# CederGroupHub/chgnet

Measured on NVIDIA H100. Metric: structures_per_sec_EFS, higher is better.
Workload: dtype f32

## Files before the change

chgnet_b200/csrc/gated_ws.cu:

```cuda
#include "gated_common.cuh"
#include "tc.cuh"

namespace chg {
namespace gated {
namespace {

constexpr int WS_THREADS = 512;
constexpr int TR = 128;
constexpr int HALF_BYTES = TR * 64 * 4;
constexpr int IMG_BYTES = 64 * 64 * 4;
constexpr int STRIP = 16;

struct WsSmem {
  static constexpr int IMG_OFF = 0;
  static constexpr int HS_OFF = 4 * IMG_BYTES;
  static constexpr int O_OFF = HS_OFF + 2 * HALF_BYTES;
  static constexpr int GIDX_OFF = O_OFF + HALF_BYTES;
  static constexpr int EIDX_OFF = GIDX_OFF + 2 * 3 * TR * 4;
  static constexpr int B2_OFF = EIDX_OFF + 4 * TR * 4;
  static constexpr int LN_OFF = B2_OFF + 128 * 4;
  static constexpr int TOTAL = LN_OFF + 256 * 4;
};

struct WsBars {
  uint64_t a_full[2], a_empty[2];
};

struct FusedArgs {
  const float* p_a;
  const float* p_b;
  const float* p_c;
  const float* wgt;
  const int32_t* idx0;
  const int32_t* idx1;
  const int32_t* idx2;
  const int32_t* ptr;
  int32_t n_rows, n_seg;
  const float* w2t;
  const float* b2;
  const float* ln;
  float* out;
  float* parts;
  float* save_pre;
  float* save_p;
};

__device__ __forceinline__ void prefetch_l2(const void* p) { asm volatile("prefetch.global.L2 [%0];" ::"l"(p)); }
__device__ __forceinline__ int swz(int r, int c) { return r * 256 + ((c ^ (r & 7)) << 4); }

__device__ __forceinline__ void build_image_ws(uint8_t* hi, uint8_t* lo, const float* __restrict__ src, int ld, int col0,
                                               int tid) {
  for (int i = tid; i < 4096; i += (int)blockDim.x) {
    const int kk = i >> 6, n = i & 63;
    uint32_t h, l;
    tc::split_tf32(__ldg(src + (size_t)kk * ld + col0 + n), h, l);
    const uint32_t off = tc::kmajor_offset(n, kk, 64);
    *reinterpret_cast<uint32_t*>(hi + off) = h;
    *reinterpret_cast<uint32_t*>(lo + off) = l;
  }
}

__device__ __forceinline__ float quad_sum(float v) {
  v += __shfl_xor_sync(0xffffffffu, v, 1);
  v += __shfl_xor_sync(0xffffffffu, v, 2);
  return v;
}
__device__ __forceinline__ void bias_ln_frag(float (&d)[32], const float* s_b2, const float* s_gamma, const float* s_beta,
                                             bool use_ln, float* save_rows, int row0, int n_rows) {
#pragma unroll
  for (int i = 0; i < 32; ++i) d[i] += s_b2[tc::frag_col(i)];
  if (save_rows != nullptr) {
#pragma unroll
    for (int i = 0; i < 32; i += 2) {
      const int g = row0 + tc::frag_row(i);
      if (g < n_rows) *reinterpret_cast<float2*>(save_rows + (size_t)g * 128 + tc::frag_col(i)) = make_float2(d[i], d[i + 1]);
    }
  }
  if (!use_ln) return;
#pragma unroll
  for (int h = 0; h < 2; ++h) {
    float s1 = 0.f;
#pragma unroll
    for (int i = 0; i < 32; ++i)
      if (((i >> 1) & 1) == h) s1 += d[i];
    const float mean = quad_sum(s1) * (1.f / 64.f);
    float s2 = 0.f;
#pragma unroll
    for (int i = 0; i < 32; ++i)
      if (((i >> 1) & 1) == h) s2 = fmaf(d[i] - mean, d[i] - mean, s2);
    const float rstd = 1.f / sqrtf(quad_sum(s2) * (1.f / 64.f) + LN_EPS);
#pragma unroll
    for (int i = 0; i < 32; ++i)
      if (((i >> 1) & 1) == h) d[i] = fmaf((d[i] - mean) * rstd, s_gamma[tc::frag_col(i)], s_beta[tc::frag_col(i)]);
  }
}

template <int MODE>
__global__ void __launch_bounds__(WS_THREADS, 1) gated_ws_fwd_kernel(const FusedArgs a) {
  extern __shared__ __align__(1024) uint8_t smem_raw[];
  uint8_t* s_img = smem_raw + WsSmem::IMG_OFF;
  uint8_t* s_hs = smem_raw + WsSmem::HS_OFF;
  uint8_t* s_o = smem_raw + WsSmem::O_OFF;
  int* s_gidx = reinterpret_cast<int*>(smem_raw + WsSmem::GIDX_OFF);
  int* s_eidx = reinterpret_cast<int*>(smem_raw + WsSmem::EIDX_OFF);
  float* s_b2 = reinterpret_cast<float*>(smem_raw + WsSmem::B2_OFF);
  float* s_ln = reinterpret_cast<float*>(smem_raw + WsSmem::LN_OFF);
  __shared__ __align__(8) WsBars bars;

  const int tid = threadIdx.x, warp = tid >> 5, lane = tid & 31;
  const bool use_ln = a.ln != nullptr;
  const int n_tiles = (a.n_rows + TR - 1) / TR;

  build_image_ws(s_img, s_img + IMG_BYTES, a.w2t, 128, 0, tid);
  build_image_ws(s_img + 2 * IMG_BYTES, s_img + 3 * IMG_BYTES, a.w2t, 128, 64, tid);
  if (tid < 128) s_b2[tid] = a.b2[tid];
  if (tid < 256) s_ln[tid] = use_ln ? a.ln[tid] : 0.f;
  if (tid == 0) {
    for (int i = 0; i < 2; ++i) {
      tc::mbar_init(&bars.a_full[i], 128);
      tc::mbar_init(&bars.a_empty[i], 256);
    }
    tc::mbar_fence_init();
  }
  tc::fence_async_smem();
  __syncthreads();

  if (warp >= 8) {
    const int half = (warp - 8) >> 2;
    const int gt = tid - 256 - half * 128;
    const int tx = gt & 15, ty = gt >> 4;
    int* gi = s_gidx + half * 3 * TR;
    uint8_t* stage = s_hs + half * HALF_BYTES;
    const int col = half * 64 + tx * 4;
    constexpr int PB = 4;
    int tl = 0;
    for (int tile = blockIdx.x; tile < n_tiles; tile += gridDim.x, ++tl) {
      const int base = tile * TR;
      {
        const int r = min(base + gt, a.n_rows - 1);
        gi[gt] = a.idx0[r];
        gi[TR + gt] = a.idx1[r];
        gi[2 * TR + gt] = a.idx2[r];
      }
      tc::wg_barrier(1 + half, 128);
      {
        const int nt = tile + gridDim.x;
        if (nt < n_tiles) {
          const int r = min(nt * TR + gt, a.n_rows - 1);
          const float* row = MODE == BOND ? a.p_c + (size_t)r * 128 + half * 64 : a.p_b + (size_t)__ldg(a.idx2 + r) * 128 + half * 64;
          prefetch_l2(row);
          prefetch_l2(row + 32);
        }
      }
#pragma unroll 1
      for (int b = 0; b < 16 / PB; ++b) {
        float4 v[PB];
#pragma unroll
        for (int i = 0; i < PB; ++i) {
          const int row = ty + 8 * (b * PB + i);
          const float* s0 = a.p_a + (size_t)gi[row] * 256 + col;
          const float* s1 = a.p_a + (size_t)gi[TR + row] * 256 + 128 + col;
          const float* s2 = a.p_b + (size_t)gi[2 * TR + row] * 128 + col;
          v[i] = ldg4(s0) + ldg4(s1) + ldg4(s2);
          if (MODE == BOND) v[i] = v[i] + ldg4(a.p_c + (size_t)min(base + row, a.n_rows - 1) * 128 + col);
        }
        if (b == 0) tc::mbar_wait(&bars.a_empty[half], (tl & 1) ^ 1);
#pragma unroll
        for (int i = 0; i < PB; ++i) {
          const int row = ty + 8 * (b * PB + i);
          if (a.save_pre != nullptr && base + row < a.n_rows) stg4(a.save_pre + (size_t)(base + row) * 128 + col, v[i]);
          *reinterpret_cast<float4*>(stage + swz(row, tx)) =
              make_float4(silu_f(v[i].x), silu_f(v[i].y), silu_f(v[i].z), silu_f(v[i].w));
        }
      }
      tc::wg_barrier(1 + half, 128);
      tc::mbar_arrive(&bars.a_full[half]);
    }
  } else {
    const int cw = warp >> 2;
    const int t = tid & 127;
    const int row0 = cw * 64;
    int* s_seg = s_eidx;
    int* s_wrow = s_eidx + TR;
    int* s_sa = s_eidx + 2 * TR;
    int* s_sb = s_eidx + 3 * TR;
    const uint32_t img = tc::smem_u32(s_img);
    int tl = 0;
    for (int tile = blockIdx.x; tile < n_tiles; tile += gridDim.x, ++tl) {
      const int base = tile * TR;
      {
        const int r = min(base + t, a.n_rows - 1);
        if (cw == 0) {
          const int seg = a.idx0[r];
          s_seg[t] = seg;
          s_sa[t] = __ldg(a.ptr + seg);
          s_sb[t] = __ldg(a.ptr + seg + 1);
        } else {
          const int wr = MODE == BOND ? a.idx1[r] : a.idx2[r];
          s_wrow[t] = wr;
          prefetch_l2(a.wgt + (size_t)wr * 64);
          prefetch_l2(a.wgt + (size_t)wr * 64 + 32);
        }
      }
      float dc[32], dg[32];
#pragma unroll
      for (int i = 0; i < 32; ++i) dc[i] = dg[i] = 0.f;
      tc::mbar_wait(&bars.a_full[0], tl & 1);
      tc::wg_gemm_k64<64>(dc, [&](int r, int k) { return *reinterpret_cast<const float*>(s_hs + swz(row0 + r, k >> 2) + (k & 3) * 4); },
                          img, img + IMG_BYTES, 2048);
      tc::mbar_arrive(&bars.a_empty[0]);
      tc::mbar_wait(&bars.a_full[1], tl & 1);
      tc::wg_gemm_k64<64>(dg, [&](int r, int k) { return *reinterpret_cast<const float*>(s_hs + HALF_BYTES + swz(row0 + r, k >> 2) + (k & 3) * 4); },
                          img + 2 * IMG_BYTES, img + 3 * IMG_BYTES, 2048);
      tc::mbar_arrive(&bars.a_empty[1]);
      float* save = a.save_p != nullptr ? a.save_p + (size_t)base * 128 : nullptr;
      bias_ln_frag(dc, s_b2, s_ln, s_ln + 64, use_ln, save, row0, a.n_rows - base);
      bias_ln_frag(dg, s_b2 + 64, s_ln + 128, s_ln + 192, use_ln, save != nullptr ? save + 64 : nullptr, row0, a.n_rows - base);
#pragma unroll
      for (int i = 0; i < 32; i += 2) {
        const int r = row0 + tc::frag_row(i), c = tc::frag_col(i);
        *reinterpret_cast<float2*>(s_o + swz(r, c >> 2) + (c & 3) * 4) =
            make_float2(silu_f(dc[i]) * sigmoid_f(dg[i]), silu_f(dc[i + 1]) * sigmoid_f(dg[i + 1]));
      }
      tc::wg_barrier(3, 256);

      const int strip_lo = base + warp * STRIP;
      const int strip_hi = min(strip_lo + STRIP, a.n_rows);
      if (strip_lo < a.n_rows) {
        float2 w[STRIP];
#pragma unroll
        for (int i = 0; i < STRIP; ++i) {
          const int rr = warp * STRIP + i;
          const float2 w0 = __ldg(reinterpret_cast<const float2*>(a.wgt + (size_t)s_wrow[rr] * 64) + lane);
          if (MODE == ATOM) {
            w[i] = w0;
          } else {
            const float2 wi = __ldg(reinterpret_cast<const float2*>(a.wgt + (size_t)s_seg[rr] * 64) + lane);
            w[i] = make_float2(wi.x * w0.x, wi.y * w0.y);
          }
        }
        float2 acc = make_float2(0.f, 0.f);
        int cur_row = warp * STRIP;
        auto emit = [&](int row0_, const float2& v) {
          const int seg = s_seg[row0_], sa = s_sa[row0_], sb = s_sb[row0_];
          float* dst;
          if (sa >= strip_lo && sb <= strip_hi) {
            dst = a.out + (size_t)seg * 64;
          } else {
            dst = a.parts + ((size_t)(strip_lo / STRIP) * 2 + (sa < strip_lo ? 0 : 1)) * 64;
          }
          *reinterpret_cast<float2*>(dst + lane * 2) = v;
        };
#pragma unroll
        for (int i = 0; i < STRIP; ++i) {
          const int rr = warp * STRIP + i;
          if (strip_lo + i < strip_hi) {
            if (s_seg[rr] != s_seg[cur_row]) {
              emit(cur_row, acc);
              cur_row = rr;
              acc = make_float2(0.f, 0.f);
            }
            const float2 o = *reinterpret_cast<const float2*>(s_o + swz(rr, lane >> 1) + (lane & 1) * 8);
            acc.x = fmaf(o.x, w[i].x, acc.x);
            acc.y = fmaf(o.y, w[i].y, acc.y);
          }
        }
        emit(cur_row, acc);
      }
      tc::wg_barrier(3, 256);
    }
  }
}

__global__ void seg_stitch_kernel(const int32_t* __restrict__ ptr, int n_seg, const float* __restrict__ parts,
                                  float* __restrict__ out) {
  const int idx = blockIdx.x * blockDim.x + threadIdx.x;
  const int s = idx >> 4, l = idx & 15;
  if (s >= n_seg) return;
  const int a = ptr[s], b = ptr[s + 1];
  if (a >= b) {
    stg4(out + (size_t)s * 64 + l * 4, make_float4(0.f, 0.f, 0.f, 0.f));
    return;
  }
  const int k0 = a / STRIP, k1 = (b - 1) / STRIP;
  if (k0 == k1) return;
  float4 acc = ldg4(parts + ((size_t)k0 * 2 + 1) * 64 + l * 4);
  for (int k = k0 + 1; k <= k1; ++k) acc = acc + ldg4(parts + ((size_t)k * 2) * 64 + l * 4);
  stg4(out + (size_t)s * 64 + l * 4, acc);
}

template <int MODE>
int launch_fused(const FusedArgs& a, cudaStream_t stream) {
  if (a.n_seg == 0) return CHG_OK;
  if (a.n_rows > 0) {
    static bool attr_set[MAX_DEVICES] = {};
    bool& set = attr_set[device_ordinal()];
    if (!set) {
      CHG_CUDA(cudaFuncSetAttribute(gated_ws_fwd_kernel<MODE>, cudaFuncAttributeMaxDynamicSharedMemorySize, WsSmem::TOTAL));
      set = true;
    }
    const int n_tiles = (a.n_rows + TR - 1) / TR;
    gated_ws_fwd_kernel<MODE><<<min(n_tiles, sm_count()), WS_THREADS, WsSmem::TOTAL, stream>>>(a);
    cudaError_t e = cudaGetLastError();
    if (e != cudaSuccess) {
      set_error("gated_ws_fwd_kernel: launch failed: %s", cudaGetErrorString(e));
      return CHG_ERR_CUDA;
    }
    count_launch();
  }
  seg_stitch_kernel<<<(a.n_seg * 16 + 255) / 256, 256, 0, stream>>>(a.ptr, a.n_seg, a.parts, a.out);
  CHG_LAUNCH_END();
}

}

int atom_conv_fused_ws(const float* pcn, const float* pe, const float* wag, const int32_t* center, const int32_t* nbr,
                       const int32_t* d2u, const int32_t* ptr_c, int n_edges, int n_atoms, const float* w2t, const float* b2,
                       const float* ln, float* agg, float* save_p, float* parts, cudaStream_t stream) {
  FusedArgs a{pcn, pe, nullptr, wag, center, nbr, d2u, ptr_c, n_edges, n_atoms, w2t, b2, ln, agg, parts, nullptr, save_p};
  return launch_fused<ATOM>(a, stream);
}

int bond_conv_fused_ws(const float* pij, const float* px, const float* pa, const float* wbg, const int32_t* ang_atom,
                       const int32_t* ang_i, const int32_t* ang_j, const int32_t* ptr_i, int n_angles, int n_slots,
                       const float* w2t, const float* b2, const float* ln, float* agg, float* save_pre, float* save_p,
                       float* parts, cudaStream_t stream) {
  FusedArgs a{pij, px, pa, wbg, ang_i, ang_j, ang_atom, ptr_i, n_angles, n_slots, w2t, b2, ln, agg, parts, save_pre, save_p};
  return launch_fused<BOND>(a, stream);
}

}
}

using namespace chg;

extern "C" int64_t chg_gated_fused_workspace_floats(int32_t n_rows) {
  if (n_rows < 0) return -1;
  const int64_t msg = (int64_t)n_rows * 64, parts = ((int64_t)n_rows + 15) / 16 * 128;
  return (msg > parts ? msg : parts) + 64;
}

extern "C" int chg_atom_conv_fused(const float* pcn, const float* pe, const float* wag, const int32_t* center,
                                   const int32_t* nbr, const int32_t* d2u, const int32_t* ptr_c, int32_t n_edges,
                                   int32_t n_atoms, const float* w2t, const float* b2, const float* ln, float* agg,
                                   float* save_p, float* work, void* stream) {
  CHG_CHECK_ARG(n_edges >= 0 && n_atoms >= 0, "negative size");
  if (n_atoms == 0) return CHG_OK;
  CHG_CHECK_ARG(ptr_c && agg, "null pointer");
  CHG_CHECK_ARG(n_edges == 0 || (pcn && pe && wag && center && nbr && d2u && w2t && b2 && work), "null pointer");
  if (gated_impl() == 3 && n_edges >= ws_min_rows())
    return gated::atom_conv_fused_ws(pcn, pe, wag, center, nbr, d2u, ptr_c, n_edges, n_atoms, w2t, b2, ln, agg, save_p, work,
                                     as_stream(stream));
  const int rc = chg_atom_conv_fwd(pcn, pe, wag, center, nbr, d2u, n_edges, w2t, b2, ln, work, save_p, nullptr, stream);
  if (rc != CHG_OK) return rc;
  return chg_segment_sum(work, 64, nullptr, ptr_c, n_atoms, n_edges, 0, agg, 64, stream);
}

extern "C" int chg_bond_conv_fused(const float* pij, const float* px, const float* pa, const float* wbg,
                                   const int32_t* ang_atom, const int32_t* ang_i, const int32_t* ang_j,
                                   const int32_t* ptr_i, int32_t n_angles, int32_t n_slots, const float* w2t,
                                   const float* b2, const float* ln, float* agg, float* save_pre, float* save_p,
                                   float* work, void* stream) {
  CHG_CHECK_ARG(n_angles >= 0 && n_slots >= 0, "negative size");
  if (n_slots == 0) return CHG_OK;
  CHG_CHECK_ARG(ptr_i && agg, "null pointer");
  CHG_CHECK_ARG(n_angles == 0 || (pij && px && pa && wbg && ang_atom && ang_i && ang_j && w2t && b2 && work), "null pointer");
  if (gated_impl() == 3 && n_angles >= ws_min_rows())
    return gated::bond_conv_fused_ws(pij, px, pa, wbg, ang_atom, ang_i, ang_j, ptr_i, n_angles, n_slots, w2t, b2, ln, agg,
                                     save_pre, save_p, work, as_stream(stream));
  const int rc = chg_bond_conv_fwd(pij, px, pa, wbg, ang_atom, ang_i, ang_j, n_angles, w2t, b2, ln, work, save_pre, save_p, stream);
  if (rc != CHG_OK) return rc;
  return chg_segment_sum(work, 64, nullptr, ptr_i, n_slots, n_angles, 0, agg, 64, stream);
}

namespace chg {
namespace gated {
namespace {

struct WsBwdSmem {
  static constexpr int IMG_OFF = 0;
  static constexpr int T1_OFF = 4 * IMG_BYTES;
  static constexpr int T2_OFF = T1_OFF + 2 * HALF_BYTES;
  static constexpr int PIDX_OFF = T2_OFF + 2 * HALF_BYTES;
  static constexpr int FIDX_OFF = PIDX_OFF + 3 * TR * 4;
  static constexpr int LN_OFF = FIDX_OFF + 3 * TR * 4;
  static constexpr int TOTAL = LN_OFF + 256 * 4;
};

struct WsBwdBars {
  uint64_t a_full, a_empty;
};

template <int MODE>
__global__ void __launch_bounds__(WS_THREADS, 1) gated_ws_bwd_kernel(const BwdArgs a) {
  extern __shared__ __align__(1024) uint8_t smem_raw[];
  uint8_t* s_img = smem_raw + WsBwdSmem::IMG_OFF;
  uint8_t* s_t1 = smem_raw + WsBwdSmem::T1_OFF;
  uint8_t* s_t2 = smem_raw + WsBwdSmem::T2_OFF;
  int* s_pidx = reinterpret_cast<int*>(smem_raw + WsBwdSmem::PIDX_OFF);
  int* s_fidx = reinterpret_cast<int*>(smem_raw + WsBwdSmem::FIDX_OFF);
  float* s_ln = reinterpret_cast<float*>(smem_raw + WsBwdSmem::LN_OFF);
  __shared__ __align__(8) WsBwdBars bars;

  const int tid = threadIdx.x, warp = tid >> 5;
  const bool use_ln = a.ln != nullptr;
  const int n_tiles = (a.n_rows + TR - 1) / TR;

  build_image_ws(s_img, s_img + IMG_BYTES, a.w2, 64, 0, tid);
  build_image_ws(s_img + 2 * IMG_BYTES, s_img + 3 * IMG_BYTES, a.w2 + 64 * 64, 64, 0, tid);
  if (tid < 256) s_ln[tid] = use_ln ? a.ln[tid] : 0.f;
  if (tid == 0) {
    tc::mbar_init(&bars.a_full, 256);
    tc::mbar_init(&bars.a_empty, 256);
    tc::mbar_fence_init();
  }
  tc::fence_async_smem();
  __syncthreads();

  if (warp < 8) {
    const int t = tid;
    const int tx = t & 15, ty = t >> 4;
    const int c0 = tx * 4;
    int tl = 0;
    for (int tile = blockIdx.x; tile < n_tiles; tile += gridDim.x, ++tl) {
      const int base = tile * TR;
      if (t < TR) {
        const int r = min(base + t, a.n_rows - 1);
        s_pidx[t] = a.idx0[r];
        s_pidx[TR + t] = a.idx1[r];
        if (MODE == ATOM) s_pidx[2 * TR + t] = a.idx2[r];
      }
      tc::wg_barrier(1, 256);
      {
        const int nt = tile + gridDim.x;
        if (nt < n_tiles) {
          const int r = min(nt * TR + (t & 127), a.n_rows - 1);
          const float* row = a.save_p + (size_t)r * 128 + (t >> 7) * 64;
          prefetch_l2(row);
          prefetch_l2(row + 32);
        }
      }
      float4 g1, g2, b1, b2v;
      if (use_ln) {
        g1 = lds4(s_ln + c0);
        b1 = lds4(s_ln + 64 + c0);
        g2 = lds4(s_ln + 128 + c0);
        b2v = lds4(s_ln + 192 + c0);
      }
      tc::mbar_wait(&bars.a_empty, (tl & 1) ^ 1);
#pragma unroll 2
      for (int pass = 0; pass < 8; ++pass) {
        const int row = pass * 16 + ty;
        const int g = base + row;
        const bool valid = g < a.n_rows;
        const int r = min(g, a.n_rows - 1);
        const float4 pc4 = ldg4(a.save_p + (size_t)r * 128 + c0);
        const float4 pg4 = ldg4(a.save_p + (size_t)r * 128 + 64 + c0);
        float4 gm, wv;
        if (MODE == ATOM) {
          gm = ldg4(a.g_in + (size_t)s_pidx[row] * 64 + c0);
          wv = ldg4(a.wgt + (size_t)s_pidx[2 * TR + row] * 64 + c0);
        } else {
          gm = ldg4(a.g_in + (size_t)s_pidx[row] * 64 + c0);
          wv = ldg4(a.wgt + (size_t)s_pidx[row] * 64 + c0);
        }
        float y1[4] = {pc4.x, pc4.y, pc4.z, pc4.w};
        float y2[4] = {pg4.x, pg4.y, pg4.z, pg4.w};
        float xh1[4], xh2[4], rstd1 = 1.f, rstd2 = 1.f;
        if (use_ln) {
          ln_stats(y1, xh1, rstd1);
          ln_stats(y2, xh2, rstd2);
#pragma unroll
          for (int j = 0; j < 4; ++j) {
            y1[j] = fmaf(xh1[j], f4at(g1, j), f4at(b1, j));
            y2[j] = fmaf(xh2[j], f4at(g2, j), f4at(b2v, j));
          }
        }
        float s1[4], core[4], gate[4];
        float4 o;
#pragma unroll
        for (int j = 0; j < 4; ++j) {
          s1[j] = sigmoid_f(y1[j]);
          core[j] = y1[j] * s1[j];
          gate[j] = sigmoid_f(y2[j]);
          f4at(o, j) = core[j] * gate[j];
        }
        float4 go;
        if (MODE == ATOM) {
          if (valid) stg4(a.g_w0 + (size_t)g * 64 + c0, gm * o);
          go = gm * wv;
        } else {
          const float4 wj = ldg4(a.wgt + (size_t)s_pidx[TR + row] * 64 + c0);
          const float4 gmo = gm * o;
          if (valid) {
            stg4(a.g_w0 + (size_t)g * 64 + c0, gmo * wj);
            stg4(a.g_w1 + (size_t)g * 64 + c0, gmo * wv);
          }
          go = gm * wv * wj;
        }
        float gy1[4], gy2[4];
#pragma unroll
        for (int j = 0; j < 4; ++j) {
          const float gj = f4at(go, j);
          gy1[j] = gj * gate[j] * (s1[j] * fmaf(y1[j], 1.f - s1[j], 1.f));
          gy2[j] = gj * core[j] * gate[j] * (1.f - gate[j]);
        }
        if (use_ln) {
          float gx[4], sa = 0.f, sb = 0.f;
#pragma unroll
          for (int j = 0; j < 4; ++j) {
            gx[j] = gy1[j] * f4at(g1, j);
            sa += gx[j];
            sb = fmaf(gx[j], xh1[j], sb);
          }
          sa = sum16(sa) * (1.f / 64.f);
          sb = sum16(sb) * (1.f / 64.f);
#pragma unroll
          for (int j = 0; j < 4; ++j) gy1[j] = rstd1 * (gx[j] - sa - xh1[j] * sb);
          sa = 0.f, sb = 0.f;
#pragma unroll
          for (int j = 0; j < 4; ++j) {
            gx[j] = gy2[j] * f4at(g2, j);
            sa += gx[j];
            sb = fmaf(gx[j], xh2[j], sb);
          }
          sa = sum16(sa) * (1.f / 64.f);
          sb = sum16(sb) * (1.f / 64.f);
#pragma unroll
          for (int j = 0; j < 4; ++j) gy2[j] = rstd2 * (gx[j] - sa - xh2[j] * sb);
        }
        *reinterpret_cast<float4*>(s_t1 + swz(row, tx)) = make_float4(gy1[0], gy1[1], gy1[2], gy1[3]);
        *reinterpret_cast<float4*>(s_t1 + HALF_BYTES + swz(row, tx)) = make_float4(gy2[0], gy2[1], gy2[2], gy2[3]);
      }
      tc::wg_barrier(1, 256);
      tc::mbar_arrive(&bars.a_full);
    }
  } else {
    const int t = tid - 256;
    const int tx = t & 15, ty = t >> 4;
    const int c0 = tx * 4;
    const int crow = t & 127, chalf = t >> 7;
    const int row0 = ((warp - 8) >> 2) * 64;
    const uint32_t img = tc::smem_u32(s_img);
    int tl = 0;
    for (int tile = blockIdx.x; tile < n_tiles; tile += gridDim.x, ++tl) {
      const int base = tile * TR;
      if (MODE == ATOM && t < TR) {
        const int r = min(base + t, a.n_rows - 1);
        s_fidx[t] = a.idx0[r];
        s_fidx[TR + t] = a.idx1[r];
        s_fidx[2 * TR + t] = a.idx2[r];
      }
      {
        const int r = min(base + crow, a.n_rows - 1);
        const float* row = MODE == ATOM ? a.p_b + (size_t)__ldg(a.idx2 + r) * 128 + chalf * 64 : a.save_pre + (size_t)r * 128 + chalf * 64;
        prefetch_l2(row);
        prefetch_l2(row + 32);
      }
      tc::mbar_wait(&bars.a_full, tl & 1);
#pragma unroll 1
      for (int half = 0; half < 2; ++half) {
        float d[32];
#pragma unroll
        for (int i = 0; i < 32; ++i) d[i] = 0.f;
        const uint8_t* src = s_t1 + half * HALF_BYTES;
        tc::wg_gemm_k64<64>(d, [&](int r, int k) { return *reinterpret_cast<const float*>(src + swz(row0 + r, k >> 2) + (k & 3) * 4); },
                            img + half * 2 * IMG_BYTES, img + (half * 2 + 1) * IMG_BYTES, 2048);
        uint8_t* dst = s_t2 + half * HALF_BYTES;
#pragma unroll
        for (int i = 0; i < 32; i += 2) {
          const int r = row0 + tc::frag_row(i), c = tc::frag_col(i);
          *reinterpret_cast<float2*>(dst + swz(r, c >> 2) + (c & 3) * 4) = make_float2(d[i], d[i + 1]);
        }
      }
      tc::mbar_arrive(&bars.a_empty);
      tc::wg_barrier(2, 256);
#pragma unroll 2
      for (int pass = 0; pass < 8; ++pass) {
        const int row = pass * 16 + ty;
        const int g = base + row;
        float4 vc, vg;
        if (MODE == ATOM) {
          const float* s0 = a.p_a + (size_t)s_fidx[row] * 256 + c0;
          const float* s1 = a.p_a + (size_t)s_fidx[TR + row] * 256 + 128 + c0;
          const float* s2 = a.p_b + (size_t)s_fidx[2 * TR + row] * 128 + c0;
          vc = ldg4(s0) + ldg4(s1) + ldg4(s2);
          vg = ldg4(s0 + 64) + ldg4(s1 + 64) + ldg4(s2 + 64);
        } else {
          const int r = min(g, a.n_rows - 1);
          vc = ldg4(a.save_pre + (size_t)r * 128 + c0);
          vg = ldg4(a.save_pre + (size_t)r * 128 + 64 + c0);
        }
        const float4 hc = *reinterpret_cast<const float4*>(s_t2 + swz(row, tx));
        const float4 hg = *reinterpret_cast<const float4*>(s_t2 + HALF_BYTES + swz(row, tx));
        if (g < a.n_rows) {
          stg4(a.g_pre + (size_t)g * 128 + c0,
               make_float4(hc.x * dsilu_f(vc.x), hc.y * dsilu_f(vc.y), hc.z * dsilu_f(vc.z), hc.w * dsilu_f(vc.w)));
          stg4(a.g_pre + (size_t)g * 128 + 64 + c0,
               make_float4(hg.x * dsilu_f(vg.x), hg.y * dsilu_f(vg.y), hg.z * dsilu_f(vg.z), hg.w * dsilu_f(vg.w)));
        }
      }
      tc::wg_barrier(2, 256);
    }
  }
}

template <int MODE>
int launch_ws_bwd(const BwdArgs& a, cudaStream_t stream) {
  if (a.n_rows == 0) return CHG_OK;
  static bool attr_set[MAX_DEVICES] = {};
  bool& set = attr_set[device_ordinal()];
  if (!set) {
    CHG_CUDA(cudaFuncSetAttribute(gated_ws_bwd_kernel<MODE>, cudaFuncAttributeMaxDynamicSharedMemorySize, WsBwdSmem::TOTAL));
    set = true;
  }
  const int n_tiles = (a.n_rows + TR - 1) / TR;
  gated_ws_bwd_kernel<MODE><<<min(n_tiles, sm_count()), WS_THREADS, WsBwdSmem::TOTAL, stream>>>(a);
  CHG_LAUNCH_END();
}

}

int atom_conv_bwd_ws(const BwdArgs& a, cudaStream_t stream) { return launch_ws_bwd<ATOM>(a, stream); }
int bond_conv_bwd_ws(const BwdArgs& a, cudaStream_t stream) { return launch_ws_bwd<BOND>(a, stream); }

}
}
```

Measured before the change: 10810.

## Double-buffer warp-specialized gated MLP stages and drop consumer block barriers

Both the forward and backward warp-specialized gated kernels now use two smem stages with per-stage mbarriers, so producers can fill tile n+1 while consumers still work on tile n. In the forward consumer, the smem output tile and the two 256-thread named barriers are replaced by a per-warp transpose buffer plus warp shuffles for segment and weight indices. Index loading is also register-prefetched one tile ahead. The backward kernel reuses the T1 buffer in place for the GEMM output, which frees smem for the second stage. This adds smem pressure and more complex phase bookkeeping, with a risk of synchronization mistakes.

```diff
diff --git a/chgnet_b200/csrc/gated_ws.cu b/chgnet_b200/csrc/gated_ws.cu
--- a/chgnet_b200/csrc/gated_ws.cu
+++ b/chgnet_b200/csrc/gated_ws.cu
@@ -14,16 +14,17 @@
 struct WsSmem {
   static constexpr int IMG_OFF = 0;
   static constexpr int HS_OFF = 4 * IMG_BYTES;
-  static constexpr int O_OFF = HS_OFF + 2 * HALF_BYTES;
-  static constexpr int GIDX_OFF = O_OFF + HALF_BYTES;
-  static constexpr int EIDX_OFF = GIDX_OFF + 2 * 3 * TR * 4;
-  static constexpr int B2_OFF = EIDX_OFF + 4 * TR * 4;
+  static constexpr int GIDX_OFF = HS_OFF + 4 * HALF_BYTES;
+  static constexpr int CIDX_OFF = GIDX_OFF + 2 * 2 * 3 * TR * 4;
+  static constexpr int OW_OFF = CIDX_OFF + 8 * 4 * 32 * 4;
+  static constexpr int OW_LD = 72;
+  static constexpr int B2_OFF = OW_OFF + 8 * 8 * OW_LD * 4;
   static constexpr int LN_OFF = B2_OFF + 128 * 4;
   static constexpr int TOTAL = LN_OFF + 256 * 4;
 };
 
 struct WsBars {
-  uint64_t a_full[2], a_empty[2];
+  uint64_t a_full[2][2], a_empty[2][2];
 };
 
 struct FusedArgs {
@@ -100,9 +101,9 @@
   extern __shared__ __align__(1024) uint8_t smem_raw[];
   uint8_t* s_img = smem_raw + WsSmem::IMG_OFF;
   uint8_t* s_hs = smem_raw + WsSmem::HS_OFF;
-  uint8_t* s_o = smem_raw + WsSmem::O_OFF;
   int* s_gidx = reinterpret_cast<int*>(smem_raw + WsSmem::GIDX_OFF);
-  int* s_eidx = reinterpret_cast<int*>(smem_raw + WsSmem::EIDX_OFF);
+  int* s_cidx = reinterpret_cast<int*>(smem_raw + WsSmem::CIDX_OFF);
+  float* s_ow = reinterpret_cast<float*>(smem_raw + WsSmem::OW_OFF);
   float* s_b2 = reinterpret_cast<float*>(smem_raw + WsSmem::B2_OFF);
   float* s_ln = reinterpret_cast<float*>(smem_raw + WsSmem::LN_OFF);
   __shared__ __align__(8) WsBars bars;
@@ -116,10 +117,11 @@
   if (tid < 128) s_b2[tid] = a.b2[tid];
   if (tid < 256) s_ln[tid] = use_ln ? a.ln[tid] : 0.f;
   if (tid == 0) {
-    for (int i = 0; i < 2; ++i) {
-      tc::mbar_init(&bars.a_full[i], 128);
-      tc::mbar_init(&bars.a_empty[i], 256);
-    }
+    for (int s = 0; s < 2; ++s)
+      for (int h = 0; h < 2; ++h) {
+        tc::mbar_init(&bars.a_full[s][h], 128);
+        tc::mbar_init(&bars.a_empty[s][h], 256);
+      }
     tc::mbar_fence_init();
   }
   tc::fence_async_smem();
@@ -129,29 +131,27 @@
     const int half = (warp - 8) >> 2;
     const int gt = tid - 256 - half * 128;
     const int tx = gt & 15, ty = gt >> 4;
-    int* gi = s_gidx + half * 3 * TR;
-    uint8_t* stage = s_hs + half * HALF_BYTES;
     const int col = half * 64 + tx * 4;
     constexpr int PB = 4;
+    int i0, i1, i2;
+    auto load_idx = [&](int tile) {
+      const int r = min(tile * TR + gt, a.n_rows - 1);
+      i0 = __ldg(a.idx0 + r);
+      i1 = __ldg(a.idx1 + r);
+      i2 = __ldg(a.idx2 + r);
+    };
+    load_idx(blockIdx.x);
     int tl = 0;
     for (int tile = blockIdx.x; tile < n_tiles; tile += gridDim.x, ++tl) {
-      const int base = tile * TR;
-      {
-        const int r = min(base + gt, a.n_rows - 1);
-        gi[gt] = a.idx0[r];
-        gi[TR + gt] = a.idx1[r];
-        gi[2 * TR + gt] = a.idx2[r];
-      }
+      const int base = tile * TR, s = tl & 1;
+      int* gi = s_gidx + (s * 2 + half) * 3 * TR;
+      uint8_t* stage = s_hs + (s * 2 + half) * HALF_BYTES;
+      gi[gt] = i0;
+      gi[TR + gt] = i1;
+      gi[2 * TR + gt] = i2;
       tc::wg_barrier(1 + half, 128);
-      {
-        const int nt = tile + gridDim.x;
-        if (nt < n_tiles) {
-          const int r = min(nt * TR + gt, a.n_rows - 1);
-          const float* row = MODE == BOND ? a.p_c + (size_t)r * 128 + half * 64 : a.p_b + (size_t)__ldg(a.idx2 + r) * 128 + half * 64;
-          prefetch_l2(row);
-          prefetch_l2(row + 32);
-        }
-      }
+      const int nt = tile + gridDim.x;
+      if (nt < n_tiles) load_idx(nt);
 #pragma unroll 1
       for (int b = 0; b < 16 / PB; ++b) {
         float4 v[PB];
@@ -164,7 +164,7 @@
           v[i] = ldg4(s0) + ldg4(s1) + ldg4(s2);
           if (MODE == BOND) v[i] = v[i] + ldg4(a.p_c + (size_t)min(base + row, a.n_rows - 1) * 128 + col);
         }
-        if (b == 0) tc::mbar_wait(&bars.a_empty[half], (tl & 1) ^ 1);
+        if (b == 0) tc::mbar_wait(&bars.a_empty[s][half], ((tl >> 1) & 1) ^ 1);
 #pragma unroll
         for (int i = 0; i < PB; ++i) {
           const int row = ty + 8 * (b * PB + i);
@@ -173,101 +173,119 @@
               make_float4(silu_f(v[i].x), silu_f(v[i].y), silu_f(v[i].z), silu_f(v[i].w));
         }
       }
-      tc::wg_barrier(1 + half, 128);
-      tc::mbar_arrive(&bars.a_full[half]);
+      tc::mbar_arrive(&bars.a_full[s][half]);
+      if (nt < n_tiles) {
+        const float* row = MODE == BOND ? a.p_c + (size_t)min(nt * TR + gt, a.n_rows - 1) * 128 + half * 64
+                                        : a.p_b + (size_t)i2 * 128 + half * 64;
+        prefetch_l2(row);
+        prefetch_l2(row + 32);
+      }
     }
   } else {
     const int cw = warp >> 2;
-    const int t = tid & 127;
     const int row0 = cw * 64;
-    int* s_seg = s_eidx;
-    int* s_wrow = s_eidx + TR;
-    int* s_sa = s_eidx + 2 * TR;
-    int* s_sb = s_eidx + 3 * TR;
+    const int g = lane >> 2, q = lane & 3;
     const uint32_t img = tc::smem_u32(s_img);
+    const int32_t* widx = MODE == BOND ? a.idx1 : a.idx2;
     int tl = 0;
     for (int tile = blockIdx.x; tile < n_tiles; tile += gridDim.x, ++tl) {
-      const int base = tile * TR;
+      const int base = tile * TR, s = tl & 1;
+      const uint32_t ph = (tl >> 1) & 1;
+      int seg[2], wrow[2];
+#pragma unroll
+      for (int h = 0; h < 2; ++h) {
+        const int r = min(base + warp * STRIP + g + 8 * h, a.n_rows - 1);
+        seg[h] = __ldg(a.idx0 + r);
+        wrow[h] = __ldg(widx + r);
+      }
+      float dc[32], dg[32];
+#pragma unroll
+      for (int i = 0; i < 32; ++i) dc[i] = dg[i] = 0.f;
+      const uint8_t* hs = s_hs + s * 2 * HALF_BYTES;
+      tc::mbar_wait(&bars.a_full[s][0], ph);
+      tc::wg_gemm_k64<64>(dc, [&](int r, int k) { return *reinterpret_cast<const float*>(hs + swz(row0 + r, k >> 2) + (k & 3) * 4); },
+                          img, img + IMG_BYTES, 2048);
+      tc::mbar_arrive(&bars.a_empty[s][0]);
       {
-        const int r = min(base + t, a.n_rows - 1);
-        if (cw == 0) {
-          const int seg = a.idx0[r];
-          s_seg[t] = seg;
-          s_sa[t] = __ldg(a.ptr + seg);
-          s_sb[t] = __ldg(a.ptr + seg + 1);
-        } else {
-          const int wr = MODE == BOND ? a.idx1[r] : a.idx2[r];
-          s_wrow[t] = wr;
-          prefetch_l2(a.wgt + (size_t)wr * 64);
-          prefetch_l2(a.wgt + (size_t)wr * 64 + 32);
-        }
-      }
-      float dc[32], dg[32];
-#pragma unroll
-      for (int i = 0; i < 32; ++i) dc[i] = dg[i] = 0.f;
-      tc::mbar_wait(&bars.a_full[0], tl & 1);
-      tc::wg_gemm_k64<64>(dc, [&](int r, int k) { return *reinterpret_cast<const float*>(s_hs + swz(row0 + r, k >> 2) + (k & 3) * 4); },
-                          img, img + IMG_BYTES, 2048);
-      tc::mbar_arrive(&bars.a_empty[0]);
-      tc::mbar_wait(&bars.a_full[1], tl & 1);
-      tc::wg_gemm_k64<64>(dg, [&](int r, int k) { return *reinterpret_cast<const float*>(s_hs + HALF_BYTES + swz(row0 + r, k >> 2) + (k & 3) * 4); },
+        const bool h = q >> 1;
+        prefetch_l2(a.wgt + (size_t)(h ? wrow[1] : wrow[0]) * 64 + (q & 1) * 32);
+        if (MODE == BOND) prefetch_l2(a.wgt + (size_t)(h ? seg[1] : seg[0]) * 64 + (q & 1) * 32);
+      }
+      int* ci = s_cidx + warp * 128 + lane;
+      ci[0] = seg[0], ci[32] = seg[1], ci[64] = wrow[0], ci[96] = wrow[1];
+      tc::mbar_wait(&bars.a_full[s][1], ph);
+      tc::wg_gemm_k64<64>(dg, [&](int r, int k) { return *reinterpret_cast<const float*>(hs + HALF_BYTES + swz(row0 + r, k >> 2) + (k & 3) * 4); },
                           img + 2 * IMG_BYTES, img + 3 * IMG_BYTES, 2048);
-      tc::mbar_arrive(&bars.a_empty[1]);
+      tc::mbar_arrive(&bars.a_empty[s][1]);
+      seg[0] = ci[0], seg[1] = ci[32], wrow[0] = ci[64], wrow[1] = ci[96];
+      int sa[2], sb[2];
+#pragma unroll
+      for (int h = 0; h < 2; ++h) {
+        sa[h] = __ldg(a.ptr + seg[h]);
+        sb[h] = __ldg(a.ptr + seg[h] + 1);
+      }
       float* save = a.save_p != nullptr ? a.save_p + (size_t)base * 128 : nullptr;
       bias_ln_frag(dc, s_b2, s_ln, s_ln + 64, use_ln, save, row0, a.n_rows - base);
       bias_ln_frag(dg, s_b2 + 64, s_ln + 128, s_ln + 192, use_ln, save != nullptr ? save + 64 : nullptr, row0, a.n_rows - base);
-#pragma unroll
-      for (int i = 0; i < 32; i += 2) {
-        const int r = row0 + tc::frag_row(i), c = tc::frag_col(i);
-        *reinterpret_cast<float2*>(s_o + swz(r, c >> 2) + (c & 3) * 4) =
-            make_float2(silu_f(dc[i]) * sigmoid_f(dg[i]), silu_f(dc[i + 1]) * sigmoid_f(dg[i + 1]));
-      }
-      tc::wg_barrier(3, 256);
-
       const int strip_lo = base + warp * STRIP;
       const int strip_hi = min(strip_lo + STRIP, a.n_rows);
-      if (strip_lo < a.n_rows) {
-        float2 w[STRIP];
-#pragma unroll
-        for (int i = 0; i < STRIP; ++i) {
-          const int rr = warp * STRIP + i;
-          const float2 w0 = __ldg(reinterpret_cast<const float2*>(a.wgt + (size_t)s_wrow[rr] * 64) + lane);
-          if (MODE == ATOM) {
-            w[i] = w0;
-          } else {
-            const float2 wi = __ldg(reinterpret_cast<const float2*>(a.wgt + (size_t)s_seg[rr] * 64) + lane);
-            w[i] = make_float2(wi.x * w0.x, wi.y * w0.y);
-          }
-        }
-        float2 acc = make_float2(0.f, 0.f);
-        int cur_row = warp * STRIP;
-        auto emit = [&](int row0_, const float2& v) {
-          const int seg = s_seg[row0_], sa = s_sa[row0_], sb = s_sb[row0_];
-          float* dst;
-          if (sa >= strip_lo && sb <= strip_hi) {
-            dst = a.out + (size_t)seg * 64;
-          } else {
-            dst = a.parts + ((size_t)(strip_lo / STRIP) * 2 + (sa < strip_lo ? 0 : 1)) * 64;
-          }
-          *reinterpret_cast<float2*>(dst + lane * 2) = v;
-        };
-#pragma unroll
-        for (int i = 0; i < STRIP; ++i) {
-          const int rr = warp * STRIP + i;
-          if (strip_lo + i < strip_hi) {
-            if (s_seg[rr] != s_seg[cur_row]) {
-              emit(cur_row, acc);
-              cur_row = rr;
+#pragma unroll
+      for (int i = 0; i < 32; ++i) dc[i] = silu_f(dc[i]) * sigmoid_f(dg[i]);
+      if (strip_lo >= a.n_rows) continue;
+
+      float2 w[STRIP];
+#pragma unroll
+      for (int i = 0; i < STRIP; ++i) {
+        const int src = 4 * (i & 7);
+        const int wr = __shfl_sync(0xffffffffu, i < 8 ? wrow[0] : wrow[1], src);
+        const float2 w0 = __ldg(reinterpret_cast<const float2*>(a.wgt + (size_t)wr * 64) + lane);
+        if (MODE == ATOM) {
+          w[i] = w0;
+        } else {
+          const int sg = __shfl_sync(0xffffffffu, i < 8 ? seg[0] : seg[1], src);
+          const float2 wi = __ldg(reinterpret_cast<const float2*>(a.wgt + (size_t)sg * 64) + lane);
+          w[i] = make_float2(wi.x * w0.x, wi.y * w0.y);
+        }
+      }
+      float2 acc = make_float2(0.f, 0.f);
+      int cur = __shfl_sync(0xffffffffu, seg[0], 0);
+      int cur_sa = __shfl_sync(0xffffffffu, sa[0], 0), cur_sb = __shfl_sync(0xffffffffu, sb[0], 0);
+      auto emit = [&]() {
+        float* dst;
+        if (cur_sa >= strip_lo && cur_sb <= strip_hi) {
+          dst = a.out + (size_t)cur * 64;
+        } else {
+          dst = a.parts + ((size_t)(strip_lo / STRIP) * 2 + (cur_sa < strip_lo ? 0 : 1)) * 64;
+        }
+        *reinterpret_cast<float2*>(dst + lane * 2) = acc;
+      };
+      float* ow = s_ow + warp * 8 * WsSmem::OW_LD;
+#pragma unroll
+      for (int h = 0; h < 2; ++h) {
+        __syncwarp();
+#pragma unroll
+        for (int j = 0; j < 8; ++j)
+          *reinterpret_cast<float2*>(ow + g * WsSmem::OW_LD + 8 * j + 2 * q) = make_float2(dc[4 * j + 2 * h], dc[4 * j + 2 * h + 1]);
+        __syncwarp();
+#pragma unroll
+        for (int i = 0; i < 8; ++i) {
+          const int rr = 8 * h + i;
+          if (strip_lo + rr < strip_hi) {
+            const int sr = __shfl_sync(0xffffffffu, h ? seg[1] : seg[0], 4 * i);
+            const int ra = __shfl_sync(0xffffffffu, h ? sa[1] : sa[0], 4 * i);
+            const int rb = __shfl_sync(0xffffffffu, h ? sb[1] : sb[0], 4 * i);
+            if (sr != cur) {
+              emit();
+              cur = sr, cur_sa = ra, cur_sb = rb;
               acc = make_float2(0.f, 0.f);
             }
-            const float2 o = *reinterpret_cast<const float2*>(s_o + swz(rr, lane >> 1) + (lane & 1) * 8);
-            acc.x = fmaf(o.x, w[i].x, acc.x);
-            acc.y = fmaf(o.y, w[i].y, acc.y);
+            const float2 o = *reinterpret_cast<const float2*>(ow + i * WsSmem::OW_LD + 2 * lane);
+            acc.x = fmaf(o.x, w[rr].x, acc.x);
+            acc.y = fmaf(o.y, w[rr].y, acc.y);
           }
         }
-        emit(cur_row, acc);
-      }
-      tc::wg_barrier(3, 256);
+      }
+      emit();
     }
   }
 }
@@ -380,15 +398,14 @@
 struct WsBwdSmem {
   static constexpr int IMG_OFF = 0;
   static constexpr int T1_OFF = 4 * IMG_BYTES;
-  static constexpr int T2_OFF = T1_OFF + 2 * HALF_BYTES;
-  static constexpr int PIDX_OFF = T2_OFF + 2 * HALF_BYTES;
+  static constexpr int PIDX_OFF = T1_OFF + 4 * HALF_BYTES;
   static constexpr int FIDX_OFF = PIDX_OFF + 3 * TR * 4;
   static constexpr int LN_OFF = FIDX_OFF + 3 * TR * 4;
   static constexpr int TOTAL = LN_OFF + 256 * 4;
 };
 
 struct WsBwdBars {
-  uint64_t a_full, a_empty;
+  uint64_t a_full[2], a_empty[2];
 };
 
 template <int MODE>
@@ -396,7 +413,6 @@
   extern __shared__ __align__(1024) uint8_t smem_raw[];
   uint8_t* s_img = smem_raw + WsBwdSmem::IMG_OFF;
   uint8_t* s_t1 = smem_raw + WsBwdSmem::T1_OFF;
-  uint8_t* s_t2 = smem_raw + WsBwdSmem::T2_OFF;
   int* s_pidx = reinterpret_cast<int*>(smem_raw + WsBwdSmem::PIDX_OFF);
   int* s_fidx = reinterpret_cast<int*>(smem_raw + WsBwdSmem::FIDX_OFF);
   float* s_ln = reinterpret_cast<float*>(smem_raw + WsBwdSmem::LN_OFF);
@@ -410,8 +426,10 @@
   build_image_ws(s_img + 2 * IMG_BYTES, s_img + 3 * IMG_BYTES, a.w2 + 64 * 64, 64, 0, tid);
   if (tid < 256) s_ln[tid] = use_ln ? a.ln[tid] : 0.f;
   if (tid == 0) {
-    tc::mbar_init(&bars.a_full, 256);
-    tc::mbar_init(&bars.a_empty, 256);
+    for (int st = 0; st < 2; ++st) {
+      tc::mbar_init(&bars.a_full[st], 256);
+      tc::mbar_init(&bars.a_empty[st], 256);
+    }
     tc::mbar_fence_init();
   }
   tc::fence_async_smem();
@@ -447,7 +465,8 @@
         g2 = lds4(s_ln + 128 + c0);
         b2v = lds4(s_ln + 192 + c0);
       }
-      tc::mbar_wait(&bars.a_empty, (tl & 1) ^ 1);
+      uint8_t* tile1 = s_t1 + (tl & 1) * 2 * HALF_BYTES;
+      tc::mbar_wait(&bars.a_empty[tl & 1], ((tl >> 1) & 1) ^ 1);
 #pragma unroll 2
       for (int pass = 0; pass < 8; ++pass) {
         const int row = pass * 16 + ty;
@@ -529,11 +548,11 @@
 #pragma unroll
           for (int j = 0; j < 4; ++j) gy2[j] = rstd2 * (gx[j] - sa - xh2[j] * sb);
         }
-        *reinterpret_cast<float4*>(s_t1 + swz(row, tx)) = make_float4(gy1[0], gy1[1], gy1[2], gy1[3]);
-        *reinterpret_cast<float4*>(s_t1 + HALF_BYTES + swz(row, tx)) = make_float4(gy2[0], gy2[1], gy2[2], gy2[3]);
+        *reinterpret_cast<float4*>(tile1 + swz(row, tx)) = make_float4(gy1[0], gy1[1], gy1[2], gy1[3]);
+        *reinterpret_cast<float4*>(tile1 + HALF_BYTES + swz(row, tx)) = make_float4(gy2[0], gy2[1], gy2[2], gy2[3]);
       }
       tc::wg_barrier(1, 256);
-      tc::mbar_arrive(&bars.a_full);
+      tc::mbar_arrive(&bars.a_full[tl & 1]);
     }
   } else {
     const int t = tid - 256;
@@ -557,23 +576,23 @@
         prefetch_l2(row);
         prefetch_l2(row + 32);
       }
-      tc::mbar_wait(&bars.a_full, tl & 1);
+      uint8_t* tile1 = s_t1 + (tl & 1) * 2 * HALF_BYTES;
+      tc::mbar_wait(&bars.a_full[tl & 1], (tl >> 1) & 1);
 #pragma unroll 1
       for (int half = 0; half < 2; ++half) {
         float d[32];
 #pragma unroll
         for (int i = 0; i < 32; ++i) d[i] = 0.f;
-        const uint8_t* src = s_t1 + half * HALF_BYTES;
+        uint8_t* src = tile1 + half * HALF_BYTES;
         tc::wg_gemm_k64<64>(d, [&](int r, int k) { return *reinterpret_cast<const float*>(src + swz(row0 + r, k >> 2) + (k & 3) * 4); },
                             img + half * 2 * IMG_BYTES, img + (half * 2 + 1) * IMG_BYTES, 2048);
-        uint8_t* dst = s_t2 + half * HALF_BYTES;
+        uint8_t* dst = src;
 #pragma unroll
         for (int i = 0; i < 32; i += 2) {
           const int r = row0 + tc::frag_row(i), c = tc::frag_col(i);
           *reinterpret_cast<float2*>(dst + swz(r, c >> 2) + (c & 3) * 4) = make_float2(d[i], d[i + 1]);
         }
       }
-      tc::mbar_arrive(&bars.a_empty);
       tc::wg_barrier(2, 256);
 #pragma unroll 2
       for (int pass = 0; pass < 8; ++pass) {
@@ -591,8 +610,8 @@
           vc = ldg4(a.save_pre + (size_t)r * 128 + c0);
           vg = ldg4(a.save_pre + (size_t)r * 128 + 64 + c0);
         }
-        const float4 hc = *reinterpret_cast<const float4*>(s_t2 + swz(row, tx));
-        const float4 hg = *reinterpret_cast<const float4*>(s_t2 + HALF_BYTES + swz(row, tx));
+        const float4 hc = *reinterpret_cast<const float4*>(tile1 + swz(row, tx));
+        const float4 hg = *reinterpret_cast<const float4*>(tile1 + HALF_BYTES + swz(row, tx));
         if (g < a.n_rows) {
           stg4(a.g_pre + (size_t)g * 128 + c0,
                make_float4(hc.x * dsilu_f(vc.x), hc.y * dsilu_f(vc.y), hc.z * dsilu_f(vc.z), hc.w * dsilu_f(vc.w)));
@@ -600,6 +619,7 @@
                make_float4(hg.x * dsilu_f(vg.x), hg.y * dsilu_f(vg.y), hg.z * dsilu_f(vg.z), hg.w * dsilu_f(vg.w)));
         }
       }
+      tc::mbar_arrive(&bars.a_empty[tl & 1]);
       tc::wg_barrier(2, 256);
     }
   }
```

Result: faster. 10990 (median of 6 runs) (+1.7%).
